# spotify-research/llark

Hardware: AMD Instinct MI355X
Metric: clips/sec (25 s audio + 128-tok prompt) end-to-end fwd (higher is better)
Workload: dtype fp16x2-split(fp32-class) prior + bf16x2-split(fp32-class) llm; 1 GPU; configs[1]+llm: 8x25s clips -> Jukebox VQ-VAE+36-layer prior -> 240x4800 -> projector -> Llama-2-7B fwd (S=371) logits; clips_per_gpu=8, global_batch=8, audio_samples=1048576, seq_len=371, prior_depth=36, prior_precision=f16x2, prior_layernorm_folded=True, parallelism=dp1 (clip-sharded, no collective), debug_overrides=False

## Files before the change

### llark_amd/csrc/llama.hip

```cpp
#include <stdlib.h>

#include "common.h"

namespace llark {

template <typename T>
__global__ void embed_gather_kernel(const long long* __restrict__ ids, const T* __restrict__ table,
                                    float* __restrict__ out, int rows, int width, int vocab, int ldo) {
    const int row = blockIdx.x;
    long long id = ids[row];
    id = id < 0 ? 0 : (id >= vocab ? vocab - 1 : id);
    const T* src = table + (size_t)id * width;
    float* dst = out + (size_t)row * ldo;
    for (int c = threadIdx.x; c < width; c += blockDim.x) dst[c] = (float)src[c];
}

template <int NV>
__global__ __launch_bounds__(256) void rmsnorm_kernel(const float* __restrict__ x, int ldx, int rows, int width,
                                                      const float* __restrict__ w, float eps,
                                                      bf16_t* __restrict__ hi, bf16_t* __restrict__ lo, int ldo) {
    const int lane = threadIdx.x & 63;
    const int row = blockIdx.x * 4 + (threadIdx.x >> 6);
    if (row >= rows) return;
    const int w4 = width >> 2;
    const float4* xr = (const float4*)(x + (size_t)row * ldx);
    const float4* w4p = (const float4*)w;
    float4 v[NV], gw[NV];
#pragma unroll
    for (int k = 0; k < NV; ++k) {
        const int c = lane + 64 * k;
        if (c < w4) {
            v[k] = xr[c];
            gw[k] = w4p[c];
        } else {
            v[k] = gw[k] = make_float4(0.f, 0.f, 0.f, 0.f);
        }
    }
    float s = 0.0f;
#pragma unroll
    for (int k = 0; k < NV; ++k)
        if (lane + 64 * k < w4) s += (v[k].x * v[k].x + v[k].y * v[k].y) + (v[k].z * v[k].z + v[k].w * v[k].w);
    const float var = wave_sum(s) / (float)width;
    const float rstd = 1.0f / sqrtf(var + eps);
    bf16x4_t* hr = (bf16x4_t*)(hi + (size_t)row * ldo);
    bf16x4_t* lr = lo ? (bf16x4_t*)(lo + (size_t)row * ldo) : nullptr;
#pragma unroll
    for (int k = 0; k < NV; ++k) {
        const int c = lane + 64 * k;
        if (c < w4) {
            const float4 g = gw[k];
            float y[4] = {g.x * (v[k].x * rstd), g.y * (v[k].y * rstd), g.z * (v[k].z * rstd), g.w * (v[k].w * rstd)};
            bf16x4_t h, l;
#pragma unroll
            for (int e = 0; e < 4; ++e) {
                h[e] = (bf16_t)y[e];
                l[e] = (bf16_t)(y[e] - (float)h[e]);
            }
            hr[c] = h;
            if (lr) lr[c] = l;
        }
    }
}

__device__ __forceinline__ void store_split(bf16_t* __restrict__ hi, bf16_t* __restrict__ lo, size_t idx, float v) {
    const bf16_t h = (bf16_t)v;
    hi[idx] = h;
    if (lo) lo[idx] = (bf16_t)(v - (float)h);
}

__global__ __launch_bounds__(256) void rope_split_kernel(const float* __restrict__ qkv, int S, int nh, int pos0,
                                                         const float* __restrict__ cos_t, const float* __restrict__ sin_t,
                                                         bf16_t* __restrict__ q, bf16_t* __restrict__ kc,
                                                         bf16_t* __restrict__ vtc, bf16_t* __restrict__ q_lo,
                                                         bf16_t* __restrict__ kc_lo, bf16_t* __restrict__ vtc_lo, int smax,
                                                         const int* __restrict__ pos_dev) {
    __shared__ float sv[64][129];
    if (pos_dev) pos0 = *pos_dev;
    const int hd = 128, H = nh * hd;
    const int s0 = blockIdx.x * 64, h = blockIdx.y, b = blockIdx.z;
    const int ns = (S - s0) < 64 ? (S - s0) : 64;
    for (int i = threadIdx.x; i < ns * 64; i += 256) {
        const int t = i >> 6, d = i & 63;
        const int s = s0 + t, pos = pos0 + s;
        const float* row = qkv + ((size_t)b * S + s) * 3 * H + h * hd;
        const float c = cos_t[(size_t)pos * 64 + d], sn = sin_t[(size_t)pos * 64 + d];
        const float q1 = row[d], q2 = row[d + 64], k1 = row[H + d], k2 = row[H + d + 64];
        const float qa = __fadd_rn(__fmul_rn(q1, c), __fmul_rn(-q2, sn));
        const float qb = __fadd_rn(__fmul_rn(q2, c), __fmul_rn(q1, sn));
        const float ka = __fadd_rn(__fmul_rn(k1, c), __fmul_rn(-k2, sn));
        const float kb = __fadd_rn(__fmul_rn(k2, c), __fmul_rn(k1, sn));
        const size_t qo = (((size_t)b * nh + h) * S + s) * hd;
        const size_t ko = (((size_t)b * nh + h) * smax + pos) * hd;
        store_split(q, q_lo, qo + d, qa);
        store_split(q, q_lo, qo + d + 64, qb);
        store_split(kc, kc_lo, ko + d, ka);
        store_split(kc, kc_lo, ko + d + 64, kb);
    }
    for (int i = threadIdx.x; i < ns * hd; i += 256) {
        const int t = i >> 7, d = i & 127;
        sv[t][d] = qkv[((size_t)b * S + s0 + t) * 3 * H + 2 * H + h * hd + d];
    }
    __syncthreads();
    for (int i = threadIdx.x; i < hd * 64; i += 256) {
        const int d = i >> 6, t = i & 63;
        if (t < ns) store_split(vtc, vtc_lo, (((size_t)b * nh + h) * hd + d) * smax + pos0 + s0 + t, sv[t][d]);
    }
}

__device__ __forceinline__ int k_swz(int key) { return ((key & 3) << 1) | (key & 8); }
__device__ __forceinline__ int k_off(int key, int chunk) { return key * 256 + ((chunk ^ k_swz(key)) << 4); }
__device__ __forceinline__ int v_off(int d, int chunk) { return d * 128 + ((chunk ^ ((d >> 1) & 7)) << 4); }
__device__ __forceinline__ int sub_row(int sub, int i) { return ((sub >> 1) << 5) + ((i >> 2) << 3) + ((sub & 1) << 2) + (i & 3); }

#ifndef ATTN_PREFILL_SM2
#define ATTN_PREFILL_SM2 1
#endif
#ifndef ATTN_PREFILL_PF
#define ATTN_PREFILL_PF 3
#endif
template <bool SPLIT, int NQ, bool P2, bool ALIBI, bool VARLEN = false>
__global__ __launch_bounds__(256) __attribute__((amdgpu_waves_per_eu((NQ == 1 && !SPLIT) ? 3 : 2, (NQ == 1 && !SPLIT) ? 3 : 2))) void attn_prefill_kernel(const bf16_t* __restrict__ q, const bf16_t* __restrict__ kc,
                                                           const bf16_t* __restrict__ vtc, const bf16_t* __restrict__ q_lo,
                                                           const bf16_t* __restrict__ kc_lo, const bf16_t* __restrict__ vtc_lo,
                                                           bf16_t* __restrict__ out, bf16_t* __restrict__ out_lo,
                                                           int S_arg, int nh, int nbh, int past, int smax, float scale,
                                                           const float* __restrict__ alibi_arg, float* __restrict__ lse, int paired,
                                                           const AttnSeqs<VARLEN> vl) {
    extern __shared__ __attribute__((aligned(16))) char smem[];
    const float* alibi = ALIBI ? alibi_arg : nullptr;
    char* sKl = smem + 32768;
    char* sVl = smem + 49152;
    constexpr int BQ = 64 * NQ;
    constexpr float LOG2E = 1.4426950408889634f;
    const int lane = threadIdx.x & 63;
    const int wv = __builtin_amdgcn_readfirstlane(threadIdx.x >> 6);
    const int g = lane >> 4, c = lane & 15;
    const int nt_grid = (S_arg + BQ - 1) / BQ;
    const int np = paired ? (nt_grid + 1) >> 1 : nt_grid;
    int pidx, bhid;
    {
        const int L = blockIdx.x;
        if ((nbh & 7) == 0) {
            bhid = (L & 7) + 8 * (L / (8 * np));
            pidx = (L >> 3) % np;
        } else {
            bhid = L / np;
            pidx = L - bhid * np;
        }
    }
    const int b = bhid / nh, h = bhid - b * nh;
    int S = S_arg, nt = nt_grid;
    size_t qrow0 = (size_t)bhid * S_arg;
    size_t krow0 = (size_t)bhid * smax;
    size_t vcol0 = (size_t)bhid * 128 * smax;
    size_t orow0 = (size_t)b * S_arg;
    if constexpr (VARLEN) {
        int off, len;
        if (!attn_seq_of(vl, b, S_arg, off, len)) return;
        S = len;
        nt = (S + BQ - 1) / BQ;
        if (pidx >= (paired ? (nt + 1) >> 1 : nt)) return;
        qrow0 = (size_t)h * vl.s_total + off;
        krow0 = (size_t)h * smax + off;
        vcol0 = (size_t)h * 128 * smax + off;
        orow0 = (size_t)off;
    }
    const int total = past + S;
    const float slope2 = alibi ? alibi[h] * LOG2E : 0.0f;
    const float scale2 = scale * LOG2E;
    const bf16_t* qb = q + qrow0 * 128;
    const bf16_t* kb = kc + krow0 * 128;
    const bf16_t* vb = vtc + vcol0;
    const bf16_t* kbl = SPLIT ? kc_lo + krow0 * 128 : nullptr;
    const bf16_t* vbl = SPLIT ? vtc_lo + vcol0 : nullptr;

    constexpr int NST = SPLIT ? 1 : 2;
    constexpr int STAGE_BYTES = 32768;
    auto stage_regs = [&](const bf16_t* kbase, const bf16_t* vbase, char* dK, char* dV, int key0) __attribute__((always_inline)) {
        int tid_ = threadIdx.x;
        if constexpr (!SPLIT) asm volatile("" : "+v"(tid_));
#pragma unroll
        for (int i = 0; i < 4; ++i) {
            const int idx = tid_ + i * 256;
            {
                const int key = idx >> 4, ch = idx & 15;
                uint4 val = make_uint4(0, 0, 0, 0);
                if (key0 + key < total) val = *(const uint4*)(kbase + (size_t)(key0 + key) * 128 + ch * 8);
                *(uint4*)(dK + k_off(key, ch)) = val;
            }
            {
                const int d = idx >> 3, ch = idx & 7;
                uint4 val = make_uint4(0, 0, 0, 0);
                const int kk = key0 + ch * 8;
                if (kk + 7 < total) {
                    val = *(const uint4*)(vbase + (size_t)d * smax + kk);
                } else if (kk < total) {
                    const bf16_t* src = vbase + (size_t)d * smax + kk;
                    unsigned short tmp[8];
#pragma unroll
                    for (int e = 0; e < 8; ++e) tmp[e] = (kk + e < total) ? ((const unsigned short*)src)[e] : (unsigned short)0;
                    val = *(uint4*)tmp;
                }
                *(uint4*)(dV + v_off(d, ch)) = val;
            }
        }
    };
    unsigned dko[4], dvo[4];
#pragma unroll
    for (int i = 0; i < 4; ++i) {
        const int j = wv * 4 + i;
        const int krow = 4 * j + (lane >> 4);
        dko[i] = (unsigned)(krow * 128 + (((lane & 15) ^ k_swz(krow)) << 3)) * 2u;
        const int d = 8 * j + (lane >> 3);
        dvo[i] = (unsigned)(d * smax + (((lane & 7) ^ ((d >> 1) & 7)) << 3)) * 2u;
    }
    auto stage_dma = [&](char* dK, char* dV, int key0) __attribute__((always_inline)) {
        const char* kt_base = (const char*)(kb + (size_t)key0 * 128);
        const char* vt_base = (const char*)(vb + key0);
#pragma unroll
        for (int i = 0; i < 4; ++i) {
            const int j = wv * 4 + i;
            __builtin_amdgcn_global_load_lds((const __attribute__((address_space(1))) void*)(kt_base + dko[i]),
                                             (__attribute__((address_space(3))) void*)(dK + j * 1024), 16, 0, 0);
            __builtin_amdgcn_global_load_lds((const __attribute__((address_space(1))) void*)(vt_base + dvo[i]),
                                             (__attribute__((address_space(3))) void*)(dV + j * 1024), 16, 0, 0);
        }
    };
    auto stage = [&](int kt) __attribute__((always_inline)) {
        const int key0 = kt * 64;
        char* base = smem + (NST == 2 ? (kt & 1) * STAGE_BYTES : 0);
        if (!SPLIT && key0 + 64 <= total) {
            stage_dma(base, base + 16384, key0);
        } else {
            stage_regs(kb, vb, base, base + 16384, key0);
            if (SPLIT) {
                __builtin_amdgcn_sched_barrier(0);
                stage_regs(kbl, vbl, sKl, sVl, key0);
            }
        }
    };
    int kaddr[4], vaddr[2];
    {
        const int krow0 = 8 * (c >> 2) + (c & 3);
#pragma unroll
        for (int ks = 0; ks < 4; ++ks) kaddr[ks] = k_off(krow0, ks * 4 + g);
#pragma unroll
        for (int p = 0; p < 2; ++p) vaddr[p] = v_off(c, p * 4 + g);
    }
    auto ksub = [](int sub) { return (32 * (sub >> 1) + 4 * (sub & 1)) * 256; };
#pragma nounroll
    for (int pass = 0; pass < 2; ++pass) {
        const int tile = pass == 0 ? nt - 1 - pidx : pidx;
        if (pass == 1 && (!paired || tile == nt - 1 - pidx)) break;
        if (pass == 1) __syncthreads();
        const int q0 = tile * BQ;
        const int wq0 = q0 + wv * 16 * NQ;
        bf16x8_t qf[NQ][4], ql[SPLIT ? NQ : 1][4];
#pragma unroll
        for (int u = 0; u < NQ; ++u) {
            int qr = wq0 + u * 16 + c;
            qr = qr < S ? qr : S - 1;
#pragma unroll
            for (int ks = 0; ks < 4; ++ks) {
                qf[u][ks] = *(const bf16x8_t*)(qb + (size_t)qr * 128 + ks * 32 + g * 8);
                if (SPLIT) ql[u][ks] = *(const bf16x8_t*)(q_lo + qrow0 * 128 + (size_t)qr * 128 + ks * 32 + g * 8);
            }
        }
        f32x4_t o[NQ][8];
        float m_run[NQ], l_run[NQ];
#pragma unroll
        for (int u = 0; u < NQ; ++u) {
#pragma unroll
            for (int dt = 0; dt < 8; ++dt) o[u][dt] = f32x4_t{0.f, 0.f, 0.f, 0.f};
            m_run[u] = -INFINITY;
            l_run[u] = 0.0f;
        }

        int last_key = past + q0 + BQ - 1;
        if (last_key > total - 1) last_key = total - 1;
        const int ntiles = last_key / 64 + 1;

        if (NST == 2) stage(0);
        for (int kt = 0; kt < ntiles; ++kt) {
            const int key0 = kt * 64;
            if (NST == 2) {
                asm volatile("s_waitcnt vmcnt(0)" ::: "memory");
                __syncthreads();
                if (kt + 1 < ntiles) stage(kt + 1);
            } else {
                __syncthreads();
                stage(kt);
                __syncthreads();
            }
            const char* sK = smem + (NST == 2 ? (kt & 1) * STAGE_BYTES : 0);
            const char* sV = sK + 16384;
            if (key0 > past + wq0 + 16 * NQ - 1) continue;
            f32x4_t st[NQ][4];
            constexpr bool PF = !SPLIT && !ALIBI && (ATTN_PREFILL_PF & 1), PFV = !SPLIT && !ALIBI && NQ == 2 && (ATTN_PREFILL_PF & 2);
            bf16x8_t vfa[PFV ? 8 : 1];
            if constexpr (PF) {
                bf16x8_t kfa[2][4];
#pragma unroll
                for (int sub = 0; sub < 4; ++sub) {
                    kfa[0][sub] = *(const bf16x8_t*)(sK + kaddr[0] + ksub(sub));
#pragma unroll
                    for (int u = 0; u < NQ; ++u) st[u][sub] = f32x4_t{0.f, 0.f, 0.f, 0.f};
                }
#pragma unroll
                for (int ks = 0; ks < 4; ++ks) {
                    __builtin_amdgcn_sched_barrier(0);
                    if (ks < 3) {
#pragma unroll
                        for (int sub = 0; sub < 4; ++sub) kfa[(ks + 1) & 1][sub] = *(const bf16x8_t*)(sK + kaddr[ks + 1] + ksub(sub));
                    }
                    __builtin_amdgcn_sched_barrier(0);
#pragma unroll
                    for (int sub = 0; sub < 4; ++sub)
#pragma unroll
                        for (int u = 0; u < NQ; ++u) st[u][sub] = __builtin_amdgcn_mfma_f32_16x16x32_bf16(kfa[ks & 1][sub], qf[u][ks], st[u][sub], 0, 0, 0);
                }
            } else {
#pragma unroll
            for (int sub = 0; sub < 4; ++sub) {
#pragma unroll
                for (int u = 0; u < NQ; ++u) st[u][sub] = f32x4_t{0.f, 0.f, 0.f, 0.f};
#pragma unroll
                for (int ks = 0; ks < 4; ++ks) {
                    const bf16x8_t kf = *(const bf16x8_t*)(sK + kaddr[ks] + ksub(sub));
                    bf16x8_t kfl;
                    if (SPLIT) kfl = *(const bf16x8_t*)(sKl + kaddr[ks] + ksub(sub));
#pragma unroll
                    for (int u = 0; u < NQ; ++u) {
                        st[u][sub] = __builtin_amdgcn_mfma_f32_16x16x32_bf16(kf, qf[u][ks], st[u][sub], 0, 0, 0);
                        if (SPLIT) {
                            st[u][sub] = __builtin_amdgcn_mfma_f32_16x16x32_bf16(kfl, qf[u][ks], st[u][sub], 0, 0, 0);
                            st[u][sub] = __builtin_amdgcn_mfma_f32_16x16x32_bf16(kf, ql[u][ks], st[u][sub], 0, 0, 0);
                        }
                    }
                }
            }
            }
            if constexpr (PFV) {
                __builtin_amdgcn_sched_barrier(0);
#pragma unroll
                for (int dt = 0; dt < 8; ++dt) vfa[dt] = *(const bf16x8_t*)(sV + vaddr[0] + dt * 2048);
                __builtin_amdgcn_sched_barrier(0);
            }
            const bool need_mask = key0 + 63 > past + wq0 || key0 + 63 >= total;
            bf16x8_t ph[NQ][2], pl[P2 ? NQ : 1][2];
            constexpr bool SM2 = !SPLIT && !P2 && !ALIBI && ATTN_PREFILL_SM2;
            if constexpr (SM2) {
#pragma unroll
                for (int u = 0; u < NQ; ++u) {
                    const int lim = past + wq0 + u * 16 + c;
                    if (need_mask) {
#pragma unroll
                        for (int sub = 0; sub < 4; ++sub)
#pragma unroll
                            for (int r = 0; r < 4; ++r) {
                                const int key = key0 + sub_row(sub, 4 * g + r);
                                if (key > lim || key >= total) st[u][sub][r] = -INFINITY;
                            }
                    }
                    float mloc = fmaxf(fmaxf(st[u][0][0], st[u][0][1]), fmaxf(st[u][0][2], st[u][0][3]));
#pragma unroll
                    for (int sub = 1; sub < 4; ++sub) mloc = fmaxf(fmaxf(fmaxf(st[u][sub][0], st[u][sub][1]), fmaxf(st[u][sub][2], st[u][sub][3])), mloc);
                    {
                        const unsigned xm = __builtin_bit_cast(unsigned, mloc);
                        const auto a = __builtin_amdgcn_permlane16_swap(xm, xm, false, false);
                        const unsigned a0 = a[0], a1 = a[1];
                        mloc = fmaxf(__builtin_bit_cast(float, a0), __builtin_bit_cast(float, a1));
                        const unsigned ym = __builtin_bit_cast(unsigned, mloc);
                        const auto b2 = __builtin_amdgcn_permlane32_swap(ym, ym, false, false);
                        const unsigned b0 = b2[0], b1 = b2[1];
                        mloc = fmaxf(__builtin_bit_cast(float, b0), __builtin_bit_cast(float, b1));
                    }
                    const float mn = fmaxf(m_run[u], mloc * scale2);
                    const bool dead = mn == -INFINITY;
                    const float alpha = dead ? 1.0f : __builtin_amdgcn_exp2f(m_run[u] - mn);
                    const float nmn = dead ? 0.0f : -mn;
                    float rs = 0.0f;
#pragma unroll
                    for (int sub = 0; sub < 4; ++sub)
#pragma unroll
                        for (int r = 0; r < 4; ++r) {
                            const float pv = __builtin_amdgcn_exp2f(__builtin_fmaf(st[u][sub][r], scale2, nmn));
                            rs += pv;
                            ph[u][sub >> 1][(sub & 1) * 4 + r] = (bf16_t)pv;
                        }
                l_run[u] = l_run[u] * alpha + rs;
                    m_run[u] = mn;
                    if (__builtin_amdgcn_ballot_w64(alpha != 1.0f) != 0) {
#pragma unroll
                        for (int dt = 0; dt < 8; ++dt)
#pragma unroll
                            for (int r = 0; r < 4; ++r) o[u][dt][r] *= alpha;
                    }
                }
            } else
#pragma unroll
            for (int u = 0; u < NQ; ++u) {
                const int lim = past + wq0 + u * 16 + c;
                float mloc = -INFINITY;
                if (need_mask || alibi) {
#pragma unroll
                    for (int sub = 0; sub < 4; ++sub)
#pragma unroll
                        for (int r = 0; r < 4; ++r) {
                            const int key = key0 + sub_row(sub, 4 * g + r);
                            float sv = st[u][sub][r] * scale2;
                            if (alibi) sv += slope2 * (float)(key - (total - 1));
                            if (key > lim || key >= total) sv = -INFINITY;
                            st[u][sub][r] = sv;
                            mloc = fmaxf(mloc, sv);
                        }
                } else {
#pragma unroll
                    for (int sub = 0; sub < 4; ++sub)
#pragma unroll
                        for (int r = 0; r < 4; ++r) {
                            st[u][sub][r] *= scale2;
                            mloc = fmaxf(mloc, st[u][sub][r]);
                        }
                }
                mloc = fmaxf(mloc, __shfl_xor(mloc, 16, 64));
                mloc = fmaxf(mloc, __shfl_xor(mloc, 32, 64));
                const float mn = fmaxf(m_run[u], mloc);
                const bool dead = mn == -INFINITY;
                const float alpha = dead ? 1.0f : __builtin_amdgcn_exp2f(m_run[u] - mn);
                float rs = 0.0f;
#pragma unroll
                for (int sub = 0; sub < 4; ++sub)
#pragma unroll
                    for (int r = 0; r < 4; ++r) {
                        const float pv = dead ? 0.0f : __builtin_amdgcn_exp2f(st[u][sub][r] - mn);
                        rs += pv;
                        const bf16_t pb = (bf16_t)pv;
                        ph[u][sub >> 1][(sub & 1) * 4 + r] = pb;
                        if (P2) pl[u][sub >> 1][(sub & 1) * 4 + r] = (bf16_t)(pv - (float)pb);
                    }
                rs += __shfl_xor(rs, 16, 64);
                rs += __shfl_xor(rs, 32, 64);
                l_run[u] = l_run[u] * alpha + rs;
                m_run[u] = mn;
                if (__builtin_amdgcn_ballot_w64(alpha != 1.0f) != 0) {
#pragma unroll
                    for (int dt = 0; dt < 8; ++dt)
#pragma unroll
                        for (int r = 0; r < 4; ++r) o[u][dt][r] *= alpha;
                }
            }
            bf16x8_t vfb[PFV ? 8 : 1];
            if constexpr (PFV) {
                __builtin_amdgcn_sched_barrier(0);
#pragma unroll
                for (int dt = 0; dt < 8; ++dt) vfb[dt] = *(const bf16x8_t*)(sV + vaddr[1] + dt * 2048);
            }
#pragma unroll
            for (int p = 0; p < 2; ++p) {
#pragma unroll
                for (int dt = 0; dt < 8; ++dt) {
                    bf16x8_t vf;
                    if constexpr (PFV) vf = p == 0 ? vfa[dt] : vfb[dt];
                    else vf = *(const bf16x8_t*)(sV + vaddr[p] + dt * 2048);
                    bf16x8_t vfl;
                    if (SPLIT) vfl = *(const bf16x8_t*)(sVl + vaddr[p] + dt * 2048);
#pragma unroll
                    for (int u = 0; u < NQ; ++u) {
                        o[u][dt] = __builtin_amdgcn_mfma_f32_16x16x32_bf16(vf, ph[u][p], o[u][dt], 0, 0, 0);
                        if (P2) o[u][dt] = __builtin_amdgcn_mfma_f32_16x16x32_bf16(vf, pl[u][p], o[u][dt], 0, 0, 0);
                        if (SPLIT) o[u][dt] = __builtin_amdgcn_mfma_f32_16x16x32_bf16(vfl, ph[u][p], o[u][dt], 0, 0, 0);
                    }
                }
            }
        }
#pragma unroll
        for (int u = 0; u < NQ; ++u) {
            const int qi = wq0 + u * 16 + c;
            if (!SPLIT && !P2 && !ALIBI && ATTN_PREFILL_SM2) {
                l_run[u] += __shfl_xor(l_run[u], 16, 64);
                l_run[u] += __shfl_xor(l_run[u], 32, 64);
            }
            if (qi >= S) continue;
            const float inv = l_run[u] > 0.0f ? 1.0f / l_run[u] : 0.0f;
            if (lse && g == 0) lse[qrow0 + qi] = (m_run[u] + log2f(l_run[u])) * 0.6931471805599453f;
            const size_t dst = (orow0 + qi) * (size_t)(nh * 128) + h * 128;
#pragma unroll
            for (int dt = 0; dt < 8; ++dt) {
                bf16x4_t hi4, lo4;
#pragma unroll
                for (int r = 0; r < 4; ++r) {
                    const float v = o[u][dt][r] * inv;
                    hi4[r] = (bf16_t)v;
                    lo4[r] = (bf16_t)(v - (float)hi4[r]);
                }
                *(bf16x4_t*)(out + dst + dt * 16 + 4 * g) = hi4;
                if (SPLIT) *(bf16x4_t*)(out_lo + dst + dt * 16 + 4 * g) = lo4;
            }
        }
    }
}

template <bool SPLIT, bool P2>
static void launch_attn_prefill(hipStream_t st, const bf16_t* q, const bf16_t* kc, const bf16_t* vtc, const bf16_t* q_lo,
                                const bf16_t* kc_lo, const bf16_t* vtc_lo, bf16_t* out, bf16_t* out_lo, int batch, int s, int nh,
                                int past, int smax, float scale, const float* alibi, float* lse) {
    const int lds = 65536;
    const int nbh = batch * nh;
    auto pairs_ok = [&](int nt) { const long wgs = (long)((nt + 1) / 2) * nbh; return nt >= 2 && (wgs >= 2048 || wgs == 512 || wgs == 1024); };
    auto go = [&](auto alibi_c) {
        constexpr bool AL = decltype(alibi_c)::value;
        auto run = [&](auto nq_c) {
            constexpr int NQ = decltype(nq_c)::value;
            const int nt = cdiv(s, 64 * NQ), pr = pairs_ok(nt);
            static PerDeviceOnce once;
            if (once.first()) (void)hipFuncSetAttribute((const void*)attn_prefill_kernel<SPLIT, NQ, P2, AL>, hipFuncAttributeMaxDynamicSharedMemorySize, lds);
            attn_prefill_kernel<SPLIT, NQ, P2, AL><<<(pr ? (nt + 1) / 2 : nt) * nbh, 256, lds, st>>>(q, kc, vtc, q_lo, kc_lo, vtc_lo, out, out_lo, s, nh, nbh, past,
                                                                                           smax, scale, alibi, lse, pr, AttnSeqs<false>{});
        };
        if (!SPLIT && (long)cdiv(s, 128) * nbh >= 1024) run(std::integral_constant<int, SPLIT ? 1 : 2>{});
        else run(std::integral_constant<int, 1>{});
    };
    if (alibi) go(std::true_type{});
    else go(std::false_type{});
}

template <int NW, int UBT>
__device__ __forceinline__ void attn_decode_body(const float* sq, float* sp, float* red, const bf16_t* kc, const bf16_t* vtc,
                                                 const bf16_t* kc_lo, const bf16_t* vtc_lo, bf16_t* __restrict__ out,
                                                 bf16_t* __restrict__ out_lo, int nh, int total, int smax, float scale,
                                                 const float* __restrict__ alibi) {
    constexpr int NT = NW * 64;
    constexpr int UB = UBT;
    constexpr int PARTS = NT / 128;
    const int h = blockIdx.x, b = blockIdx.y;
    const size_t bh = (size_t)b * nh + h;
    const int tid = threadIdx.x, lane = tid & 63, wv = tid >> 6;
    __syncthreads();
    const bf16_t* kb = kc + bh * (size_t)smax * 128;
    const bf16_t* kbl = kc_lo ? kc_lo + bh * (size_t)smax * 128 : nullptr;
    const int chunk = lane & 15, sub = lane >> 4;
    float qv[8];
#pragma unroll
    for (int e = 0; e < 8; ++e) qv[e] = sq[chunk * 8 + e];
    float lmax = -INFINITY;
    constexpr int KSTEP = NW * 4;
    for (int jb = wv * 4 + sub; jb < total + KSTEP - 1; jb += KSTEP * UB) {
        bf16x8_t kv[UB], kl[UB];
#pragma unroll
        for (int u = 0; u < UB; ++u) {
            int j = jb + KSTEP * u;
            j = j < total ? j : total - 1;
            kv[u] = *(const bf16x8_t*)(kb + (size_t)j * 128 + chunk * 8);
            if (kbl) kl[u] = *(const bf16x8_t*)(kbl + (size_t)j * 128 + chunk * 8);
        }
#pragma unroll
        for (int u = 0; u < UB; ++u) {
            const int j = jb + KSTEP * u;
            float s = 0.0f;
            if (kbl) {
#pragma unroll
                for (int e = 0; e < 8; ++e) s = fmaf(qv[e], (float)kv[u][e] + (float)kl[u][e], s);
            } else {
#pragma unroll
                for (int e = 0; e < 8; ++e) s = fmaf(qv[e], (float)kv[u][e], s);
            }
            s += __shfl_xor(s, 1, 64);
            s += __shfl_xor(s, 2, 64);
            s += __shfl_xor(s, 4, 64);
            s += __shfl_xor(s, 8, 64);
            s *= scale;
            if (alibi) s += alibi[blockIdx.x] * (float)(j - (total - 1));
            if (j < total) {
                if (chunk == 0) sp[j] = s;
                lmax = fmaxf(lmax, s);
            }
        }
    }
    lmax = wave_max(lmax);
    if (lane == 0) red[wv] = lmax;
    __syncthreads();
    float mx = red[0];
#pragma unroll
    for (int i = 1; i < NW; ++i) mx = fmaxf(mx, red[i]);
    float lsum = 0.0f;
    const int tpad = (total + 7) & ~7;
    for (int j = tid; j < tpad; j += NT) {
        float p = 0.0f;
        if (j < total) {
            p = expf(sp[j] - mx);
            lsum += p;
        }
        sp[j] = p;
    }
    lsum = wave_sum(lsum);
    __syncthreads();
    if (lane == 0) red[NW + wv] = lsum;
    __syncthreads();
    float tot = 0.0f;
#pragma unroll
    for (int i = 0; i < NW; ++i) tot += red[NW + i];
    const float inv = 1.0f / tot;
    const int d = tid / PARTS, part = tid % PARTS;
    const bf16_t* vr = vtc + (bh * 128 + d) * (size_t)smax;
    const bf16_t* vrl = vtc_lo ? vtc_lo + (bh * 128 + d) * (size_t)smax : nullptr;
    float acc = 0.0f;
    for (int cb = part * 8; cb < tpad; cb += 8 * PARTS * UB) {
        bf16x8_t vv[UB], vl[UB];
#pragma unroll
        for (int u = 0; u < UB; ++u) {
            int c8 = cb + 8 * PARTS * u;
            c8 = c8 < tpad ? c8 : tpad - 8;
            vv[u] = *(const bf16x8_t*)(vr + c8);
            if (vrl) vl[u] = *(const bf16x8_t*)(vrl + c8);
        }
#pragma unroll
        for (int u = 0; u < UB; ++u) {
            const int c8 = cb + 8 * PARTS * u;
            if (c8 < tpad) {
                if (vrl && c8 + 8 > total) {
#pragma unroll
                    for (int e = 0; e < 8; ++e)
                        if (c8 + e < total) acc = fmaf(sp[c8 + e], (float)vv[u][e] + (float)vl[u][e], acc);
                } else if (vrl) {
#pragma unroll
                    for (int e = 0; e < 8; ++e) acc = fmaf(sp[c8 + e], (float)vv[u][e] + (float)vl[u][e], acc);
                } else {
#pragma unroll
                    for (int e = 0; e < 8; ++e) acc = fmaf(sp[c8 + e], (float)vv[u][e], acc);
                }
            }
        }
    }
#pragma unroll
    for (int o = 1; o < PARTS; o <<= 1) acc += __shfl_xor(acc, o, 64);
    if (part == 0) store_split(out, out_lo, (size_t)b * (nh * 128) + h * 128 + d, acc * inv);
}

template <int NW, int UBT, bool ROWS = false>
__global__ __launch_bounds__(NW * 64, (NW >= 16 && UBT == 4) ? 7 : 1) void attn_decode_kernel(const bf16_t* __restrict__ q, bf16_t* kc, bf16_t* vtc,
                                                              const bf16_t* __restrict__ q_lo, bf16_t* kc_lo, bf16_t* vtc_lo,
                                                              bf16_t* __restrict__ out, bf16_t* __restrict__ out_lo,
                                                              int nh, int total, int smax, float scale,
                                                              const int* __restrict__ pos_dev, const float* __restrict__ alibi,
                                                              const float* __restrict__ qkv, const float* __restrict__ cos_t,
                                                              const float* __restrict__ sin_t, unsigned* chain_done) {
    extern __shared__ __attribute__((aligned(16))) char smem[];
    if constexpr (ROWS) {
        const int p = pos_dev[blockIdx.y];
        if (p < 0 || p >= smax) {
            if (threadIdx.x < 128)
                store_split(out, out_lo, (size_t)blockIdx.y * (nh * 128) + blockIdx.x * 128 + threadIdx.x, 0.0f);
            return;
        }
        total = p + 1;
    } else if (pos_dev) total = *pos_dev + 1;
    float* sp = (float*)smem;
    __shared__ float sq[128];
    __shared__ float red[2 * NW];
    const int h = blockIdx.x, b = blockIdx.y;
    const size_t bh = (size_t)b * nh + h;
    const int tid = threadIdx.x, lane = tid & 63, wv = tid >> 6;
    if (qkv) {
        const int pos = total - 1, H = nh * 128;
        const float* row = qkv + (size_t)b * 3 * H + h * 128;
        const bool split = kc_lo != nullptr;
        if (tid < 64) {
            const int d = tid;
            const float c = cos_t[(size_t)pos * 64 + d], sn = sin_t[(size_t)pos * 64 + d];
            const float q1 = row[d], q2 = row[d + 64], k1 = row[H + d], k2 = row[H + d + 64];
            const float qa = __fadd_rn(__fmul_rn(q1, c), __fmul_rn(-q2, sn));
            const float qb = __fadd_rn(__fmul_rn(q2, c), __fmul_rn(q1, sn));
            const float ka = __fadd_rn(__fmul_rn(k1, c), __fmul_rn(-k2, sn));
            const float kb2 = __fadd_rn(__fmul_rn(k2, c), __fmul_rn(k1, sn));
            const bf16_t ha = (bf16_t)qa, hb = (bf16_t)qb;
            sq[d] = (float)ha + (split ? (float)(bf16_t)(qa - (float)ha) : 0.0f);
            sq[d + 64] = (float)hb + (split ? (float)(bf16_t)(qb - (float)hb) : 0.0f);
            const size_t ko = (bh * (size_t)smax + pos) * 128;
            store_split(kc, kc_lo, ko + d, ka);
            store_split(kc, kc_lo, ko + d + 64, kb2);
        } else if (tid >= 128 && tid < 256) {
            const int d = tid - 128;
            store_split(vtc, vtc_lo, (bh * 128 + d) * (size_t)smax + pos, row[2 * H + d]);
        }
    } else if (tid < 128) {
        sq[tid] = (float)q[bh * 128 + tid] + (q_lo ? (float)q_lo[bh * 128 + tid] : 0.0f);
    }
    attn_decode_body<NW, UBT>(sq, sp, red, kc, vtc, kc_lo, vtc_lo, out, out_lo, nh, total, smax, scale, alibi);
    chain_signal(ChainSync{nullptr, 0u, chain_done});
}

__device__ __forceinline__ float clamp_keep_nan(float v, float lim) {
    return (lim > 0.0f && v == v) ? fminf(fmaxf(v, -lim), lim) : v;
}

template <int NW, int UBT>
__global__ __launch_bounds__(NW * 64, (NW >= 16 && UBT == 4) ? 7 : 1) void mpt_attn_decode_kernel(
    const float* __restrict__ qkv, int ldq, int nh, const int* __restrict__ pos_rows, float clip, const float* __restrict__ q_ln_w,
    const float* __restrict__ q_ln_b, const float* __restrict__ k_ln_w, const float* __restrict__ k_ln_b, float eps, bf16_t* kc, bf16_t* vtc,
    bf16_t* kc_lo, bf16_t* vtc_lo, int smax, bf16_t* __restrict__ out, bf16_t* __restrict__ out_lo, float scale,
    const float* __restrict__ alibi) {
    extern __shared__ __attribute__((aligned(16))) char smem[];
    const int pos = pos_rows[blockIdx.y];
    if (pos < 0 || pos >= smax) {
        if (threadIdx.x < 128) store_split(out, out_lo, (size_t)blockIdx.y * (nh * 128) + blockIdx.x * 128 + threadIdx.x, 0.0f);
        return;
    }
    float* sp = (float*)smem;
    __shared__ float sq[128];
    __shared__ float red[2 * NW];
    __shared__ float stat[4];
    const int h = blockIdx.x, b = blockIdx.y, H = nh * 128;
    const size_t bh = (size_t)b * nh + h;
    const int tid = threadIdx.x, lane = tid & 63, wv = tid >> 6;
    const float* row = qkv + (size_t)b * ldq;
    const bool ln = q_ln_w != nullptr, split = kc_lo != nullptr;
    const int d = tid & 127, isk = tid >> 7;
    float x = 0.0f, g = 1.0f, be = 0.0f;
    if (tid < 256) {
        x = clamp_keep_nan(row[isk * H + h * 128 + d], clip);
        if (ln) {
            g = (isk ? k_ln_w : q_ln_w)[h * 128 + d];
            const float* bp = isk ? k_ln_b : q_ln_b;
            be = bp ? bp[h * 128 + d] : 0.0f;
        }
    }
    if (tid >= 128 && tid < 256)
        store_split(vtc, vtc_lo, (bh * 128 + d) * (size_t)smax + pos, clamp_keep_nan(row[2 * H + h * 128 + d], clip));
    if (ln) {
        if (wv < 2) {
            const float4* xr = (const float4*)(row + wv * H);
            const int w4 = H >> 2;
            float s = 0.0f;
            for (int c = lane; c < w4; c += 64) {
                float4 v = xr[c];
                v.x = clamp_keep_nan(v.x, clip), v.y = clamp_keep_nan(v.y, clip), v.z = clamp_keep_nan(v.z, clip), v.w = clamp_keep_nan(v.w, clip);
                s += (v.x + v.y) + (v.z + v.w);
            }
            const float mean = wave_sum(s) / (float)H;
            float q = 0.0f;
            for (int c = lane; c < w4; c += 64) {
                float4 v = xr[c];
                v.x = clamp_keep_nan(v.x, clip), v.y = clamp_keep_nan(v.y, clip), v.z = clamp_keep_nan(v.z, clip), v.w = clamp_keep_nan(v.w, clip);
                const float a = v.x - mean, bb = v.y - mean, cc = v.z - mean, dd = v.w - mean;
                q += (a * a + bb * bb) + (cc * cc + dd * dd);
            }
            const float rstd = 1.0f / sqrtf(wave_sum(q) / (float)H + eps);
            if (lane == 0) stat[2 * wv] = mean, stat[2 * wv + 1] = rstd;
        }
        __syncthreads();
        if (tid < 256) x = (x - stat[2 * isk]) * stat[2 * isk + 1] * g + be;
    }
    if (tid < 128) {
        const bf16_t hi = (bf16_t)x;
        sq[d] = (float)hi + (split ? (float)(bf16_t)(x - (float)hi) : 0.0f);
    } else if (tid < 256) {
        store_split(kc, kc_lo, (bh * (size_t)smax + pos) * 128 + d, x);
    }
    attn_decode_body<NW, UBT>(sq, sp, red, kc, vtc, kc_lo, vtc_lo, out, out_lo, nh, pos + 1, smax, scale, alibi);
}

enum AttnDecodePos { POS_HOST, POS_DEV, POS_ROWS };
struct AttnDecodeArgs {
    const char* name;
    bool fused;
    const void *q, *q_lo;
    const float *qkv, *cos_t, *sin_t, *alibi;
    void *k_cache, *vt_cache, *k_cache_lo, *vt_cache_lo, *out, *out_lo;
    int batch, nh, hd, smax, max_pos;
    AttnDecodePos from;
    long total;
    const int *pos_dev, *pos_rows;
    unsigned* chain_done;
    llark_stream_t stream;
};

static int attn_decode(const AttnDecodeArgs& a) {
    LLARK_REQUIRE(a.k_cache && a.vt_cache && a.out && (a.fused ? a.qkv && a.cos_t && a.sin_t : a.q != nullptr) &&
                      (a.from == POS_HOST || (a.from == POS_DEV ? a.pos_dev : a.pos_rows)), "%s: null pointer", a.name);
    LLARK_REQUIRE(a.hd == 128, "%s: head_dim must be 128 (Llama-2), got %d", a.name, a.hd);
    LLARK_REQUIRE(!a.fused || ((a.k_cache_lo == nullptr) == (a.vt_cache_lo == nullptr) && (a.k_cache_lo == nullptr) == (a.out_lo == nullptr)),
                  "%s: give all lo planes (fp32-class mode) or none", a.name);
    bool ok = a.batch > 0 && a.nh > 0 && a.smax % 8 == 0;
    if (a.from == POS_HOST) ok = ok && a.total > 0 && a.total <= a.smax && (!a.fused || a.total <= a.max_pos);
    if (a.from == POS_DEV) ok = ok && (a.fused || a.smax > 0);
    if (a.from == POS_ROWS) ok = ok && a.smax > 0 && a.smax <= a.max_pos;
    LLARK_REQUIRE(ok, "%s: bad shape batch=%d nh=%d pos=%ld smax=%d max_pos=%d", a.name, a.batch, a.nh, a.total - 1, a.smax, a.max_pos);
    const size_t lds = (a.from == POS_HOST ? (size_t)((a.total + 7) & ~7L) : (size_t)a.smax) * sizeof(float);
    LLARK_REQUIRE(lds <= 128 * 1024, "%s: context too long for the LDS score buffer (total=%ld smax=%d)", a.name, a.total, a.smax);
    const float scale = (float)(1.0 / sqrt((double)a.hd));
    const int total = a.from == POS_HOST ? (int)a.total : 1;
    auto go = [&](auto rows_c) {
        constexpr bool ROWS = decltype(rows_c)::value;
        auto launch = [&](auto kern, int threads) {
            kern<<<dim3(a.nh, a.batch), threads, lds, (hipStream_t)a.stream>>>(
                (const bf16_t*)a.q, (bf16_t*)a.k_cache, (bf16_t*)a.vt_cache, (const bf16_t*)a.q_lo, (bf16_t*)a.k_cache_lo, (bf16_t*)a.vt_cache_lo,
                (bf16_t*)a.out, (bf16_t*)a.out_lo, a.nh, total, a.smax, scale, ROWS ? a.pos_rows : a.pos_dev, a.alibi, a.qkv, a.cos_t, a.sin_t, a.chain_done);
        };
        static PerDeviceOnce once;
        const bool first = once.first();
        if (lds > 48 * 1024 && (first || (int)lds > once.slot())) {
            (void)hipFuncSetAttribute((const void*)attn_decode_kernel<4, 8, ROWS>, hipFuncAttributeMaxDynamicSharedMemorySize, (int)lds);
            (void)hipFuncSetAttribute((const void*)attn_decode_kernel<16, 4, ROWS>, hipFuncAttributeMaxDynamicSharedMemorySize, (int)lds);
            once.slot() = (int)lds;
        }
        if ((long)a.nh * a.batch < 256) launch(attn_decode_kernel<16, 4, ROWS>, 1024);
        else launch(attn_decode_kernel<4, 8, ROWS>, 256);
    };
    if (a.from == POS_ROWS) go(std::true_type{});
    else go(std::false_type{});
    return check_launch(a.name);
}

__global__ __launch_bounds__(256) void ce_rows_kernel(const float* __restrict__ logits, int ldl, int S, int vocab,
                                                      const long long* __restrict__ labels, long long ignore_index,
                                                      float* __restrict__ row_loss) {
    __shared__ float red[8];
    const int s = blockIdx.x, b = blockIdx.y;
    const int row = b * S + s;
    const int lane = threadIdx.x & 63, wv = threadIdx.x >> 6;
    long long tgt = (s + 1 < S) ? labels[(size_t)b * S + s + 1] : ignore_index;
    if (tgt == ignore_index || tgt < 0 || tgt >= vocab) {
        if (threadIdx.x == 0) row_loss[row] = CE_ROW_NOT_COUNTED;
        return;
// ... 375 lines not shown
```

Before: 13.66 clips/s.

## Register-prefetch next K/V tile in split-precision attention prefill

Adds a PIPE path for the split (hi/lo bf16) attention prefill kernel. It loads the next 64-key K/V tile (hi and lo) into registers while the current tile is computed, then writes it into LDS with masking for the ragged last tile. This overlaps global loads with MMA work in place of the synchronous stage-then-compute sequence. The path is on by default for SPLIT and can be turned off with an environment variable. The cost is 16 extra uint4 registers per thread, which may hurt occupancy or cause spills.

Result: no change. 13.71 clips/s (median of 6 runs) (+0.3%).

```diff
diff --git a/llark_amd/csrc/llama.hip b/llark_amd/csrc/llama.hip
--- a/llark_amd/csrc/llama.hip
+++ b/llark_amd/csrc/llama.hip
@@ -118,7 +118,7 @@
 #ifndef ATTN_PREFILL_PF
 #define ATTN_PREFILL_PF 3
 #endif
-template <bool SPLIT, int NQ, bool P2, bool ALIBI, bool VARLEN = false>
+template <bool SPLIT, int NQ, bool P2, bool ALIBI, bool VARLEN = false, bool PIPE = SPLIT>
 __global__ __launch_bounds__(256) __attribute__((amdgpu_waves_per_eu((NQ == 1 && !SPLIT) ? 3 : 2, (NQ == 1 && !SPLIT) ? 3 : 2))) void attn_prefill_kernel(const bf16_t* __restrict__ q, const bf16_t* __restrict__ kc,
                                                            const bf16_t* __restrict__ vtc, const bf16_t* __restrict__ q_lo,
                                                            const bf16_t* __restrict__ kc_lo, const bf16_t* __restrict__ vtc_lo,
@@ -226,6 +226,48 @@
                                              (__attribute__((address_space(3))) void*)(dV + j * 1024), 16, 0, 0);
         }
     };
+    auto fetch_tile = [&](int key0, uint4 (&rk)[4], uint4 (&rv)[4], uint4 (&rkl)[4], uint4 (&rvl)[4]) __attribute__((always_inline)) {
+        const int tid_ = threadIdx.x;
+        const int vlast = (total - 1) & ~7;
+#pragma unroll
+        for (int i = 0; i < 4; ++i) {
+            const int idx = tid_ + i * 256;
+            int key = key0 + (idx >> 4), kk = key0 + (idx & 7) * 8;
+            key = key < total ? key : total - 1;
+            kk = kk < vlast ? kk : vlast;
+            const unsigned ko = (unsigned)key * 128u + (unsigned)(idx & 15) * 8u;
+            const unsigned vo = (unsigned)(idx >> 3) * (unsigned)smax + (unsigned)kk;
+            rk[i] = *(const uint4*)(kb + ko);
+            rv[i] = *(const uint4*)(vb + vo);
+            rkl[i] = *(const uint4*)(kbl + ko);
+            rvl[i] = *(const uint4*)(vbl + vo);
+        }
+    };
+    auto put_tile = [&](int key0, const uint4 (&rk)[4], const uint4 (&rv)[4], const uint4 (&rkl)[4], const uint4 (&rvl)[4]) __attribute__((always_inline)) {
+        const int tid_ = threadIdx.x;
+        const bool ragged = key0 + 64 > total;
+#pragma unroll
+        for (int i = 0; i < 4; ++i) {
+            const int idx = tid_ + i * 256;
+            uint4 k4 = rk[i], v4 = rv[i], kl4 = rkl[i], vl4 = rvl[i];
+            if (ragged) {
+                if (key0 + (idx >> 4) >= total) k4 = kl4 = make_uint4(0, 0, 0, 0);
+                const int live = total - (key0 + (idx & 7) * 8);
+                if (live < 8) {
+                    const unsigned mx = live > 1 ? 0xffffffffu : live > 0 ? 0x0000ffffu : 0u;
+                    const unsigned my = live > 3 ? 0xffffffffu : live > 2 ? 0x0000ffffu : 0u;
+                    const unsigned mz = live > 5 ? 0xffffffffu : live > 4 ? 0x0000ffffu : 0u;
+                    const unsigned mw = live > 6 ? 0x0000ffffu : 0u;
+                    v4 = make_uint4(v4.x & mx, v4.y & my, v4.z & mz, v4.w & mw);
+                    vl4 = make_uint4(vl4.x & mx, vl4.y & my, vl4.z & mz, vl4.w & mw);
+                }
+            }
+            *(uint4*)(smem + k_off(idx >> 4, idx & 15)) = k4;
+            *(uint4*)(smem + 16384 + v_off(idx >> 3, idx & 7)) = v4;
+            *(uint4*)(sKl + k_off(idx >> 4, idx & 15)) = kl4;
+            *(uint4*)(sVl + v_off(idx >> 3, idx & 7)) = vl4;
+        }
+    };
     auto stage = [&](int kt) __attribute__((always_inline)) {
         const int key0 = kt * 64;
         char* base = smem + (NST == 2 ? (kt & 1) * STAGE_BYTES : 0);
@@ -280,10 +322,18 @@
         if (last_key > total - 1) last_key = total - 1;
         const int ntiles = last_key / 64 + 1;
 
+        uint4 nk[PIPE ? 4 : 1], nv[PIPE ? 4 : 1], nkl[PIPE ? 4 : 1], nvl[PIPE ? 4 : 1];
         if (NST == 2) stage(0);
+        if constexpr (PIPE) fetch_tile(0, nk, nv, nkl, nvl);
         for (int kt = 0; kt < ntiles; ++kt) {
             const int key0 = kt * 64;
-            if (NST == 2) {
+            if constexpr (PIPE) {
+                __syncthreads();
+                put_tile(key0, nk, nv, nkl, nvl);
+                __syncthreads();
+                if (kt + 1 < ntiles) fetch_tile(key0 + 64, nk, nv, nkl, nvl);
+                __builtin_amdgcn_sched_barrier(0);
+            } else if (NST == 2) {
                 asm volatile("s_waitcnt vmcnt(0)" ::: "memory");
                 __syncthreads();
                 if (kt + 1 < ntiles) stage(kt + 1);
@@ -501,6 +551,11 @@
     }
 }
 
+static bool split_one_stage() {
+    const char* e = getenv("LLARK_ATTN_SPLIT_PIPE");
+    return e && e[0] == '0';
+}
+
 template <bool SPLIT, bool P2>
 static void launch_attn_prefill(hipStream_t st, const bf16_t* q, const bf16_t* kc, const bf16_t* vtc, const bf16_t* q_lo,
                                 const bf16_t* kc_lo, const bf16_t* vtc_lo, bf16_t* out, bf16_t* out_lo, int batch, int s, int nh,
@@ -510,16 +565,18 @@
     auto pairs_ok = [&](int nt) { const long wgs = (long)((nt + 1) / 2) * nbh; return nt >= 2 && (wgs >= 2048 || wgs == 512 || wgs == 1024); };
     auto go = [&](auto alibi_c) {
         constexpr bool AL = decltype(alibi_c)::value;
-        auto run = [&](auto nq_c) {
+        auto run = [&](auto nq_c, auto pipe_c) {
             constexpr int NQ = decltype(nq_c)::value;
+            constexpr bool PIPE = decltype(pipe_c)::value;
             const int nt = cdiv(s, 64 * NQ), pr = pairs_ok(nt);
             static PerDeviceOnce once;
-            if (once.first()) (void)hipFuncSetAttribute((const void*)attn_prefill_kernel<SPLIT, NQ, P2, AL>, hipFuncAttributeMaxDynamicSharedMemorySize, lds);
-            attn_prefill_kernel<SPLIT, NQ, P2, AL><<<(pr ? (nt + 1) / 2 : nt) * nbh, 256, lds, st>>>(q, kc, vtc, q_lo, kc_lo, vtc_lo, out, out_lo, s, nh, nbh, past,
+            if (once.first()) (void)hipFuncSetAttribute((const void*)attn_prefill_kernel<SPLIT, NQ, P2, AL, false, PIPE>, hipFuncAttributeMaxDynamicSharedMemorySize, lds);
+            attn_prefill_kernel<SPLIT, NQ, P2, AL, false, PIPE><<<(pr ? (nt + 1) / 2 : nt) * nbh, 256, lds, st>>>(q, kc, vtc, q_lo, kc_lo, vtc_lo, out, out_lo, s, nh, nbh, past,
                                                                                            smax, scale, alibi, lse, pr, AttnSeqs<false>{});
         };
-        if (!SPLIT && (long)cdiv(s, 128) * nbh >= 1024) run(std::integral_constant<int, SPLIT ? 1 : 2>{});
-        else run(std::integral_constant<int, 1>{});
+        if (!SPLIT && (long)cdiv(s, 128) * nbh >= 1024) run(std::integral_constant<int, SPLIT ? 1 : 2>{}, std::false_type{});
+        else if (SPLIT && !split_one_stage()) run(std::integral_constant<int, 1>{}, std::integral_constant<bool, SPLIT>{});
+        else run(std::integral_constant<int, 1>{}, std::false_type{});
     };
     if (alibi) go(std::true_type{});
     else go(std::false_type{});
```
